# jinhan/tacotron2-vae

Measured on AMD Instinct MI355X. Metric: mel-frames/s (train step, batch=6, 80-mel), higher is better.
Workload: dtype f32; 1 GPU; configs[1]: Tacotron2-VAE fp32 train step (fwd+loss+bwd+clip+Adam), B=6/GPU fixed shape T_in=84 T_out=400, dropout on, random-init seed 1234; step_mode=hip-graph replay, decoder_forward=persistent, decoder_backward=persistent, startup_steps=43, global_batch=6, parallelism=dp1

## Files before the change

### include/t2vae.h

```cpp
#ifndef T2VAE_H
#define T2VAE_H
#include <stdint.h>
#ifdef __cplusplus
extern "C" {
#endif

#define T2V_OK 0
#define T2V_ERR_DIMS -1
#define T2V_ERR_ARG -2
#define T2V_ERR_LAUNCH -3

const char* t2v_version(void);
const char* t2v_last_error(void);

void t2v_set_phase_profile(unsigned long long* dev_buf32);
int t2v_stamp(unsigned long long* dev_buf, int slot, void* stream);
int t2v_debug_spin(int wgs, int microseconds, void* stream);

typedef struct t2v_step_params {
    uint64_t epoch;
    float lr;
    float bc1;
    float bc2s;
    float kl_weight;
// ... 208 lines not shown

typedef struct t2v_dec_items {
    int32_t* stop_item;
    const uint64_t* item_seeds;
} t2v_dec_items;
int t2v_decoder_infer_steps_items(const t2v_dec_weights* w, const t2v_dec_infer_bufs* s, int B, int T_in,
                                  int t_begin, int t_end, float gate_threshold, float p_prenet,
                                  int external_prenet, uint64_t seed, const t2v_dec_items* items, void* stream);
int t2v_decoder_infer_persistent_items(const t2v_dec_persist_weights* w, const t2v_dec_persist_bufs* s, int B, int T_in,
                                       int t_end, float gate_threshold, float p_prenet, uint64_t seed,
                                       const t2v_dec_items* items, void* stream);

typedef struct t2v_dec_window {
    int32_t back;
    int32_t ahead;
} t2v_dec_window;
int t2v_decoder_infer_steps_window(const t2v_dec_weights* w, const t2v_dec_infer_bufs* s, int B, int T_in,
                                   int t_begin, int t_end, float gate_threshold, float p_prenet,
                                   int external_prenet, uint64_t seed, const t2v_dec_items* items,
                                   const t2v_dec_window* window, void* stream);
int t2v_decoder_infer_persistent_window(const t2v_dec_persist_weights* w, const t2v_dec_persist_bufs* s, int B, int T_in,
                                        int t_end, float gate_threshold, float p_prenet, uint64_t seed,
                                        const t2v_dec_items* items, const t2v_dec_window* window, void* stream);

int t2v_conv1d_stat_blocks(int B, int T, int Cin, int Cout, int KS);
int t2v_conv1d_stat_blocks_bf16(int B, int T, int Cin, int Cout, int KS);
long long t2v_conv1d_staged_launches(void);
int t2v_conv1d_fwd(const float* W, const float* X, const float* bias, float* Y, float* stat_part,
                   int B, int Cin, int T, int Cout, int KS, void* stream);
int t2v_conv1d_dw_scratch_floats(int B, int Cin, int T, int Cout, int KS);
int t2v_conv1d_bwd(const float* W, const float* X, const float* dY, float* dX, float* dW, float* Wt_scratch,
                   float* dw_scratch,
                   int B, int Cin, int T, int Cout, int KS, void* stream);
int t2v_conv1d_flip_weights(const float* const* W, float* const* Wt, const int* Cout, const int* Cin, int KS, int n,
                            void* stream);
int t2v_conv1d_fwd_bf16(const float* W, const float* X, const float* bias, float* Y, float* stat_part,
                        void* Wp_scratch, int B, int Cin, int T, int Cout, int KS, void* stream);
int t2v_conv1d_bwd_bf16(const float* W, const float* X, const float* dY, float* dX, float* dW,
                        void* Wp_scratch, float* dw_scratch, int B, int Cin, int T, int Cout, int KS, void* stream);

int t2v_bn_act_fwd(const float* y, const float* stat_part, int nblk, const float* gamma, const float* beta,
                   float* running_mean, float* running_var, float* mean_out, float* rstd_out, float* out,
                   int B, int M, int T, int act, int training, float p_drop, float momentum, float eps,
                   uint64_t seed, uint32_t rng_stream, uint32_t rng_t, void* stream);
int t2v_bn_act_fwd_len(const float* y, const float* gamma, const float* beta, const float* running_mean,
                       const float* running_var, float* out, const int32_t* lengths, int B, int M, int T, int act, float eps,
                       void* stream);
int t2v_bn_act_bwd(const float* y, const float* dout, const float* mean, const float* rstd,
                   const float* gamma, const float* beta, float* dy, float* dgamma, float* dbeta,
                   float* dconv_bias, int B, int M, int T, int act, float p_drop, uint64_t seed,
                   uint32_t rng_stream, uint32_t rng_t, void* stream);
int t2v_bn_act_bwd_eval(const float* y, const float* dout, const float* mean, const float* rstd,
                   const float* gamma, const float* beta, float* dy, float* dgamma, float* dbeta,
                   float* dconv_bias, int B, int M, int T, int act, float p_drop, uint64_t seed,
                   uint32_t rng_stream, uint32_t rng_t, void* stream);
int t2v_bn_act_slices(int backward, int B, int M, int T, int training, int has_partials);

int t2v_embedding_fwd(const long long* ids, const float* W, float* out_bct, int B, int T, int C, int n_symbols, void* stream);
int t2v_embedding_bwd(const long long* ids, const float* dy_bct, float* dW, int B, int T, int C, int n_symbols, void* stream);

int t2v_gemm_epilogue_bwd(const float* dy, const float* y, float* out, size_t n, float scale, void* stream);

long t2v_colsum_scratch_floats(long M, long N);
int t2v_colsum(const float* A, long lda, long M, long N, float* scratch, float* out, void* stream);

int t2v_mask_outputs(float* mel, float* mel_post, float* gate, const int* lengths, int B, int C, int T, float gate_fill,
                     void* stream);
int t2v_mask_time(const float* x, float* out, const int32_t* lengths, int B, int C, int T, void* stream);
int t2v_reparam_fwd(const float* eps, const float* mu, const float* logvar, float* z, long n, void* stream);
int t2v_reparam_bwd(const float* dz, const float* eps, const float* logvar, float* dlogvar, long n, void* stream);
int t2v_gather_words(const void* const* src, void* const* dst, int n, void* stream);
int t2v_concat2_rows(const float* a, long lda, int na, const float* b, long ldb, int nb, float* out, long rows, void* stream);

int t2v_bilstm_fwd(const float* gx, const float* whh, const int32_t* lengths, float* y, float* gates,
                   float* cells, float* hx_scratch, uint32_t* sync3, int B, int T, void* stream);
int t2v_bilstm_bwd(const float* whh, const int32_t* lengths, const float* dy, const float* gates,
                   const float* cells, float* dg, float* dgx_scratch, uint32_t* sync3, int B, int T,
                   void* stream);

int t2v_gemm_f32(const float* A, long sAi, long sAk, const float* B, long sBj, long sBk, const float* bias,
                 float* C, int ldc, int M, int N, int K, int relu, int accumulate, float p_drop,
                 uint64_t seed, uint32_t rng_stream, uint32_t rng_t, void* stream);
long t2v_gemm_splitk_scratch_floats(int M, int N, int K);
int t2v_gemm_f32_splitk(const float* A, long sAi, long sAk, const float* B, long sBj, long sBk, const float* bias,
                        float* C, int ldc, int M, int N, int K, int relu, int accumulate, float p_drop,
                        uint64_t seed, uint32_t rng_stream, uint32_t rng_t, float* splitk_scratch, void* stream);

int t2v_gemm_f32_set_mode(int x3);

typedef struct t2v_gemm_group {
    const float* A;
    long sAi;
    long sAk;
    int nb;
    const float* B[3];
    long sBj[3];
    long sBk[3];
    int N[3];
    float* C[3];
    int ldc[3];
} t2v_gemm_group;
long t2v_gemm_f32_grouped_scratch_floats(const t2v_gemm_group* groups, int ngroups, int M, int K);
int t2v_gemm_f32_grouped(const t2v_gemm_group* groups, int ngroups, int M, int K, int accumulate, float* scratch, void* stream);
long t2v_gemm_f32_grouped_group_offset(const t2v_gemm_group* groups, int ngroups, int M, int K, int g);
int t2v_gemm_f32_grouped_handed(const t2v_gemm_group* groups, int ngroups, int M, int K, int accumulate, float* scratch, int handed,
                                const uint32_t* done_ctr, int done_cap, void* stream);
long t2v_gemm_bf16_grouped_scratch_floats(const t2v_gemm_group* groups, int ngroups, int M, int K);
int t2v_gemm_bf16_grouped(const t2v_gemm_group* groups, int ngroups, int M, int K, int accumulate, float* scratch, void* stream);

int t2v_conv1d_x3_set_mode(int mode);
int t2v_conv1d_takes_x3(int B, int Cin, int T, int Cout, int KS, int bf16);
#define T2V_CONV_OP_FWD 0
#define T2V_CONV_OP_DX 1
#define T2V_CONV_OP_DW 2
#define T2V_CONV_ROUTE_GEMM 0
#define T2V_CONV_ROUTE_FWD 1
#define T2V_CONV_ROUTE_FWD_DMA 2
#define T2V_CONV_ROUTE_X3 3
#define T2V_CONV_ROUTE_BF16 4
#define T2V_CONV_ROUTE_BF16K32 5
#define T2V_CONV_ROUTE_PLANE1 6
#define T2V_CONV_ROUTE_DW 7
#define T2V_CONV_ROUTE_DW_BF16 8
#define T2V_CONV_ROUTES 9
int t2v_conv1d_route(int op, int B, int Cin, int T, int Cout, int KS, int bf16, int w_mod16, int* fallback, int* tile, int* ksplit,
                     int* dw_splits, int* stat_blocks, int* dw_scratch_floats, int* plane_splits, int* plane_chunk);
const char* t2v_conv1d_route_name(int route);

int t2v_gemm_f32_batched(const float* A, long sAb, long sAi, long sAk, const float* B, long sBb, long sBj, long sBk,
                         float* C, long sCb, int ldc, int nbatch, int M, int N, int K, void* stream);
int t2v_gemm_bf16(const float* A, long sAi, long sAk, const float* B, long sBj, long sBk, const float* bias,
                  float* C, int ldc, int M, int N, int K, int relu, int accumulate, float p_drop,
                  uint64_t seed, uint32_t rng_stream, uint32_t rng_t, void* stream);
long t2v_gemm_bf16_splitk_scratch_floats(int M, int N, int K);
int t2v_gemm_bf16_splitk(const float* A, long sAi, long sAk, const float* B, long sBj, long sBk, const float* bias,
                         float* C, int ldc, int M, int N, int K, int relu, int accumulate, float p_drop,
                         uint64_t seed, uint32_t rng_stream, uint32_t rng_t, float* splitk_scratch, void* stream);

#define T2V_GEMM_ROUTE_F32_64 0
#define T2V_GEMM_ROUTE_F32_64_SPLITK 1
#define T2V_GEMM_ROUTE_F32_BIG_128 2
#define T2V_GEMM_ROUTE_F32_BIG_64 3
#define T2V_GEMM_ROUTE_F32_X3 4
#define T2V_GEMM_ROUTE_BF16_64 5
#define T2V_GEMM_ROUTE_BF16_64_SPLITK 6
#define T2V_GEMM_ROUTE_BF16_BIG 7
#define T2V_GEMM_ROUTE_BF16_BIG_SPLITK 8
#define T2V_GEMM_ROUTE_BF16_PLANES 9
#define T2V_GEMM_ROUTE_BF16_TO_F32_BIG 10
#define T2V_GEMM_ROUTES 11
int t2v_gemm_route(int M, int N, int K, long sAi, long sAk, long sBj, long sBk, int a_mod16, int b_mod16, int scratch_mod16,
                   int has_scratch, int relu, float p_drop, int bf16, int* form, int* splits, int* k_per_split);
const char* t2v_gemm_route_name(int route);


int t2v_conv2d_s2_fwd(const float* x, const float* w, const float* bias, float* y, int B, int Cx, int H, int W,
                      int Cout, int coord, void* stream);
int t2v_conv2d_s2_dw_scratch_floats(int B, int Cx, int H, int W, int Cout, int coord);
int t2v_conv2d_s2_bwd(const float* x, const float* w, const float* dy, float* dx, float* dw, float* dw_scratch,
                      int B, int Cx, int H, int W, int Cout, int coord, void* stream);

long t2v_conv2d_s2_gemm_scratch_floats(int B, int Cx, int H, int W, int Cout, int coord);
int t2v_conv2d_s2_fwd_gemm(const float* x, const float* w, const float* bias, float* y, float* scratch, int B, int Cx, int H, int W,
                           int Cout, int coord, void* stream);
int t2v_conv2d_s2_bwd_gemm(const float* x, const float* w, const float* dy, float* dx, float* dw, float* scratch, int B, int Cx, int H,
                           int W, int Cout, int coord, void* stream);
int t2v_gru_fwd(const float* gi, const float* whh, const float* bhh, float* hs, float* gsave, float* xchg,
                uint32_t* sync2, int B, int T, void* stream);
int t2v_gru_bwd(const float* whh, const float* hs, const float* gsave, const float* dh_last, float* dgi,
                float* dgh, float* xchg, uint32_t* sync2, int B, int T, void* stream);

int t2v_conv2d_s2_fwd_ragged(const float* x, const float* w, const float* bias, float* y, const int32_t* hlen, int B, int Cx,
                             int H, int W, int Cout, int coord, int x_tstride, void* stream);
long t2v_conv2d_s2_gemm_ragged_scratch_floats(int B, int Cx, int H, int W, int Cout, int coord);
int t2v_conv2d_s2_fwd_gemm_ragged(const float* x, const float* w, const float* bias, float* y, float* scratch,
                                  const int32_t* hlen, int B, int Cx, int H, int W, int Cout, int coord, int x_tstride,
                                  void* stream);
int t2v_gru_fwd_len(const float* gi, const float* whh, const float* bhh, float* hs, float* gsave, float* xchg,
                    uint32_t* sync2, const int32_t* steps, float* h_last, int B, int T, void* stream);
int t2v_loss_fwd_bwd(const float* mel, const float* post, const float* mel_t, const float* gate,
                     const float* gate_t, const float* mu, const float* logvar, float* dmel, float* dpost,
                     float* dgate, float* dmu, float* dlogvar, float* part192, float* out4, uint32_t* ticket,
                     uint64_t n_mel, int n_gate, int n_lat, float kl_weight, void* stream);

int t2v_clip_adam_step(float* params, float* grads, float* exp_avg, float* exp_avg_sq, uint64_t n,
                       float lr, float beta1, float beta2, float eps, float weight_decay,
                       float max_norm, float inv_world, float bc1, float bc2, float* partials,
                       float* norm_out, void* stream);
int t2v_clip_adam_step_guarded(float* params, float* grads, float* exp_avg, float* exp_avg_sq, uint64_t n,
                               float lr, float beta1, float beta2, float eps, float weight_decay,
                               float max_norm, float inv_world, float bc1, float bc2, float* partials,
                               float* norm_out, const uint32_t* guard, int guard_n, void* stream);
int t2v_clip_adam_ema_step_guarded(float* params, float* grads, float* exp_avg, float* exp_avg_sq, uint64_t n,
                                   float lr, float beta1, float beta2, float eps, float weight_decay,
                                   float max_norm, float inv_world, float bc1, float bc2, float* partials,
                                   float* norm_out, const uint32_t* guard, int guard_n, float* ema, float ema_rate,
                                   int ema_warmup, uint64_t ema_t, void* stream);

int t2v_mel_frontend(const float* wav_f32, const int16_t* wav_i16, const int64_t* n_samples, int B,
                     int n_stride, float scale, int n_fft, int hop, int n_mel, const float* window,
                     const float* tw512, const float* tw1024, const int32_t* mel_start,
                     const int32_t* mel_len, const float* mel_w, int maxw, float* mel_out,
                     int t_stride, void* stream);

int t2v_stft_polar(const float* wav, const int64_t* n_samples, int B, int n_stride, int n_fft, int hop,
                   const float* window, const float* tw512, const float* tw1024, float* mag, float* phase,
                   int t_stride, void* stream);
size_t t2v_istft_scratch_bytes(int B, int t_stride);
int t2v_istft(const float* mag, const float* phase, const int32_t* n_frames, int B, int t_stride, int n_fft, int hop,
              const float* window, const float* tw512, const float* tw1024, void* scratch, float* out, int out_stride,
              void* stream);
size_t t2v_griffin_lim_scratch_bytes(int B, int t_stride);
int t2v_griffin_lim(const float* mag, const float* angles, const int32_t* n_frames, int B, int t_stride, int n_fft,
                    int hop, int n_iters, const float* window, const float* tw512, const float* tw1024, void* scratch,
                    float* out, int out_stride, void* stream);
int t2v_mel_to_magnitude(const float* mel, const float* pinv_basis, const int32_t* n_frames, int B, int t_stride,
                         int n_mel, float* mag, void* stream);
size_t t2v_griffin_lim_fast_scratch_bytes(int B, int t_stride);
int t2v_griffin_lim_fast(const float* mag, const float* angles, const int32_t* n_frames, int B, int t_stride, int n_fft,
                         int hop, int n_iters, float momentum, const float* window, const float* tw512,
                         const float* tw1024, void* scratch, float* out, int out_stride, void* stream);
int t2v_mel_to_magnitude_nnls(const float* mel, const float* pinv_basis, const int32_t* tap_lo, const float* tap_w0,
                              const float* tap_w1, const int32_t* filt_start, const int32_t* filt_len, float lipschitz,
                              int n_iters, const int32_t* n_frames, int B, int t_stride, int n_mel, float* mag,
                              void* stream);

#define T2V_DTW_MAX_FRAMES 2048
size_t t2v_mel_dtw_scratch_bytes(int B, int tx_max, int ty_max);
int t2v_mel_dtw(const float* X, const int32_t* nx, int x_stride, const float* Y, const int32_t* ny, int y_stride,
                int B, int n_mel, float* dist, void* scratch, void* stream);

#define T2V_TSNE_MAX_POINTS 16384
#define T2V_TSNE_EXAG_ITERS 250
size_t t2v_tsne_scratch_bytes(int N, int D);
int t2v_tsne_affinities(const float* X, int N, int D, float perplexity, float* P, void* scratch, void* stream);
int t2v_tsne_gradient(const float* P, const float* Y, int N, float exaggeration, float* grad, float* kl_or_null,
                      void* scratch, void* stream);
int t2v_tsne_run(const float* P, float* Y_inout, int N, int n_iter, float learning_rate, float* kl_trace, void* scratch,
                 void* stream);

#define T2V_F0_MAX_LAG 400
int t2v_f0_yin(const float* y, const int32_t* n, int y_stride, int B, int tau_min, int tau_max, float threshold, float* f0,
               float* aperiodicity, int out_stride, void* stream);

#define T2V_ALIGN_FRAMES 16
size_t t2v_alignment_scratch_bytes(int B, int N, int T_in);
int t2v_alignment_stats(const float* A, long long a_stride_b, long long a_stride_t, const int32_t* n_frames,
                        const int32_t* n_text, int B, int N, int T_in, int max_jump, float cover_min, int32_t* path,
                        int path_stride, float* mass, int mass_stride, float* focus, int32_t* stats, void* scratch,
                        void* stream);

#define T2V_RESAMPLE_MAX_TAPS 32768
int t2v_resample(const void* x, int x_is_pcm16, float scale, const int32_t* n, int x_stride, int B, const float* taps, int up,
                 int down, int half, float* y, int out_stride, void* stream);
int t2v_trim_bounds(const float* y, const int32_t* n, int y_stride, int B, float top_db, int pad_frames, float* ms, int ms_stride,
                    int32_t* bounds, void* stream);
int t2v_crop_rows(const float* y, int y_stride, const int32_t* bounds, int B, void* out, int out_is_pcm16, int out_stride,
                  int32_t* stats, void* stream);

#define T2V_LATENT_MAX_POINTS 16384
#define T2V_LATENT_MAX_CLASSES 8
#define T2V_LATENT_MAX_K 32
#define T2V_LATENT_TILE 128
size_t t2v_latent_scratch_bytes(int N, int M, int C, int k, int slice_rows);
int t2v_latent_neighbours(const float* R, const int32_t* labels, int N, int D, int C, const float* Q, int M,
                          const int32_t* exclude, const int32_t* target, int k, int slice_rows, int32_t* nn_idx,
                          float* nn_dist, float* class_sum, int32_t* class_cnt, int32_t* rank, void* scratch, void* stream);

#define T2V_NCEP 13
#define T2V_ALIGNED_COUNTS 4
#define T2V_ALIGNED_SUMS 8
int t2v_mel_cepstrum(const float* M, const int32_t* n, int m_stride, int B, int n_mel, int n_cep, const float* table, float* out,
                     int out_stride, void* stream);
size_t t2v_cep_dtw_scratch_bytes(int B, int tx_max, int ty_max);
int t2v_cep_dtw_forward(const float* X, const int32_t* nx, int x_stride, const float* Y, const int32_t* ny, int y_stride, int B,
                        int n_cep, float* dist, void* scratch, void* stream);
int t2v_cep_dtw_walk(const int32_t* nx, int x_stride, const int32_t* ny, int y_stride, int B, const void* scratch, int32_t* K,
                     int32_t* path, int path_stride, void* stream);
int t2v_cep_dtw_path(const float* X, const int32_t* nx, int x_stride, const float* Y, const int32_t* ny, int y_stride, int B,
                     int n_cep, float* dist, int32_t* K, int32_t* path, int path_stride, void* scratch, void* stream);
int t2v_path_scores(const int32_t* path, const int32_t* K, int path_stride, const float* X, const int32_t* nx, int x_stride,
                    const float* Y, const int32_t* ny, int y_stride, const float* fx, int fx_stride, const float* fy, int fy_stride,
                    int B, int n_cep, int32_t* counts, float* sums, void* stream);

#define T2V_LOUDNESS_CHUNK 64
#define T2V_LOUDNESS_TILE 16384
size_t t2v_loudness_scratch_bytes(int B, int y_stride, int hop);
int t2v_loudness(const float* y, const int32_t* n, int y_stride, int B, const double* table, int hop, float* frame_ms,
                 int ms_stride, float* block_pw, int blk_stride, int32_t* rows, void* scratch, void* stream);
int t2v_scale_rows(float* y, const int32_t* n, int y_stride, int B, const float* gains, void* stream);

#define T2V_TSM_BINS 513
#define T2V_TSM_MAX_RATIO 1023
#define T2V_TSM_MAX_FRAMES (1 << 20)
size_t t2v_phase_vocoder_scratch_bytes(int B, int out_stride, int phase_lock);
int t2v_phase_vocoder(const float* mag, const float* phase, const int32_t* n_frames, int B, int T, int t_stride, int num, int den,
                      int phase_lock, float* mag_out, float* phase_out, int out_stride, void* scratch, void* stream);

size_t t2v_spsi_scratch_bytes(int B, int t_stride);
int t2v_spsi(const float* mag, const int32_t* n_frames, int B, int T, int t_stride, float* phase_out, void* scratch, void* stream);

#define T2V_ENV_BINS 513
#define T2V_ENV_MAX_ORDER 256
#define T2V_ENV_MAX_ITERS 32
int t2v_spectral_envelope(const float* mag, const int32_t* n_frames, int B, int T, int t_stride, int order, int iters, int p, int q,
                          float* log_env_out, float* mag_out, int out_stride, void* stream);
// ... 26 lines not shown
```

### tacotron2-vae_amd/csrc/gemm.hip

```cpp
#include <stdlib.h>
#include <string.h>
#include "t2v_common.h"
#include "t2v_kernels.h"
#include "t2v_coop.h"
#include "t2v_x3.h"
#include "t2v_xchg.h"
#include "gemm_x3_tile.h"

#define GM_BM 64
#define GM_BN 64
#define GM_BK 32

struct GemmArgs {
    const float* A; const float* B; const float* bias; float* C;
    long sAi, sAk, sBj, sBk;
    int M, N, K, ldc;
    int relu, accumulate;
    float p_drop; uint64_t seed; uint32_t rng_stream, rng_t;
    const t2v_step_params* step;
    int kz_chunk;
    float* part;
    int nbatch;
    long sAb, sBb, sCb;
    int nsub;
    long sAs, sBs;
    int bias_row;
    unsigned* tile_ctr;
};

__device__ __forceinline__ void gemm64_epilogue(const GemmArgs& a, f32x16& acc, int i0, int j0, int wm, int wn, int lane, int tid) {
    const int j = j0 + 32 * wn + (lane & 31);
    if (a.part) {
        if (j < a.N) {
#pragma unroll
            for (int r = 0; r < 16; ++r) {
                const int i = i0 + 32 * wm + (r & 3) + 8 * (r >> 2) + 4 * (lane >> 5);
                if (i < a.M) st_sc1(a.part + ((size_t)blockIdx.z * a.M + i) * a.N + j, acc[r]);
            }
        }
        __shared__ unsigned last_;
        asm volatile("s_waitcnt vmcnt(0)" ::: "memory");
        __syncthreads();
        unsigned* ctr = a.tile_ctr + blockIdx.y * gridDim.x + blockIdx.x;
        if (tid == 0) last_ = __hip_atomic_fetch_add(ctr, 1u, __ATOMIC_RELAXED, __HIP_MEMORY_SCOPE_AGENT) == gridDim.z - 1 ? 1u : 0u;
        __syncthreads();
        if (!last_) return;
        if (tid == 0) __hip_atomic_store(ctr, 0u, __ATOMIC_RELAXED, __HIP_MEMORY_SCOPE_AGENT);
        const int nz = (int)gridDim.z;
#pragma unroll
        for (int r = 0; r < 16; ++r) acc[r] = 0.f;
        if (j < a.N) {
            for (int z0 = 0; z0 < nz; z0 += 4) {
                float v[4][16];
#pragma unroll
                for (int u = 0; u < 4; ++u) {
                    const int z = min(z0 + u, nz - 1);
#pragma unroll
                    for (int r = 0; r < 16; ++r) {
                        const int i = min(i0 + 32 * wm + (r & 3) + 8 * (r >> 2) + 4 * (lane >> 5), a.M - 1);
                        v[u][r] = ld_sc1(a.part + ((size_t)z * a.M + i) * a.N + j);
                    }
                }
#pragma unroll
                for (int u = 0; u < 4; ++u)
                    if (z0 + u < nz) {
#pragma unroll
                        for (int r = 0; r < 16; ++r) acc[r] += v[u][r];
                    }
            }
        }
    }
    if (j < a.N) {
        const float bv = (a.bias && !a.bias_row) ? a.bias[j] : 0.f;
#pragma unroll
        for (int r = 0; r < 16; ++r) {
            const int i = i0 + 32 * wm + (r & 3) + 8 * (r >> 2) + 4 * (lane >> 5);
            if (i < a.M) {
                const size_t idx = (size_t)i * a.ldc + j;
                float v = acc[r] + ((a.bias && a.bias_row) ? a.bias[i] : bv);
                if (a.accumulate) v += a.C[idx];
                if (a.relu) v = fmaxf(v, 0.f);
                if (a.p_drop > 0.f) v *= t2v_drop_scale(t2v_step_seed(a.seed, a.step), a.rng_stream, a.rng_t, (uint32_t)idx, a.p_drop);
                a.C[idx] = v;
            }
        }
    }
}

template <bool A_KC, bool B_KC>
__global__ __launch_bounds__(256) void k_gemm_f32(GemmArgs a) {
    __shared__ float As[2][GM_BK][GM_BM + 1];
    __shared__ float Bs[2][GM_BK][GM_BN + 1];
    const int tid = threadIdx.x, wave = tid >> 6, lane = tid & 63;
    const int wm = wave >> 1, wn = wave & 1;
    const int i0 = blockIdx.y * GM_BM, j0 = blockIdx.x * GM_BN;
    if (a.nbatch > 1) {
        const int zb = a.nsub > 1 ? blockIdx.z / a.nsub : blockIdx.z, zs = a.nsub > 1 ? blockIdx.z - zb * a.nsub : 0;
        a.A += zb * a.sAb + zs * a.sAs; a.B += zb * a.sBb + zs * a.sBs; a.C += blockIdx.z * a.sCb;
    }
    const int kbeg = a.kz_chunk ? blockIdx.z * a.kz_chunk : 0, kend = a.kz_chunk ? min(a.K, kbeg + a.kz_chunk) : a.K;
    constexpr int NE = GM_BM * GM_BK / 256;
    float ra[NE], rb[NE];
    auto load_tiles = [&](int k0) {
#pragma unroll
        for (int e8 = 0; e8 < NE; ++e8) {
            const int e = tid + 256 * e8;
            {
                const int kk = A_KC ? (e & (GM_BK - 1)) : (e >> 6);
                const int ii = A_KC ? (e >> 5) : (e & (GM_BM - 1));
                const int i = i0 + ii, k = k0 + kk;
                ra[e8] = (i < a.M && k < kend) ? a.A[(long)i * a.sAi + (long)k * a.sAk] : 0.f;
            }
            {
                const int kk = B_KC ? (e & (GM_BK - 1)) : (e >> 6);
                const int jj = B_KC ? (e >> 5) : (e & (GM_BN - 1));
                const int j = j0 + jj, k = k0 + kk;
                rb[e8] = (j < a.N && k < kend) ? a.B[(long)j * a.sBj + (long)k * a.sBk] : 0.f;
            }
        }
    };
    auto store_tiles = [&](int buf) {
#pragma unroll
        for (int e8 = 0; e8 < NE; ++e8) {
            const int e = tid + 256 * e8;
            if (A_KC) As[buf][e & (GM_BK - 1)][e >> 5] = ra[e8]; else As[buf][e >> 6][e & (GM_BM - 1)] = ra[e8];
            if (B_KC) Bs[buf][e & (GM_BK - 1)][e >> 5] = rb[e8]; else Bs[buf][e >> 6][e & (GM_BN - 1)] = rb[e8];
        }
    };
    f32x16 acc;
#pragma unroll
    for (int r = 0; r < 16; ++r) acc[r] = 0.f;
    const int nkt = (kend - kbeg + GM_BK - 1) / GM_BK;
    load_tiles(kbeg);
    store_tiles(0);
    __syncthreads();
    const int ai = 32 * wm + (lane & 31), bj = 32 * wn + (lane & 31), kh = lane >> 5;
    for (int kt = 0; kt < nkt; ++kt) {
        const int buf = kt & 1;
        if (kt + 1 < nkt) load_tiles(kbeg + (kt + 1) * GM_BK);
#pragma unroll
        for (int s = 0; s < GM_BK / 2; ++s)
            acc = __builtin_amdgcn_mfma_f32_32x32x2f32(As[buf][2 * s + kh][ai], Bs[buf][2 * s + kh][bj], acc, 0, 0, 0);
        if (kt + 1 < nkt) store_tiles(buf ^ 1);
        __syncthreads();
    }
    gemm64_epilogue(a, acc, i0, j0, wm, wn, lane, tid);
}

#include "t2v_ring.h"
#define GM_CTR_RING ((size_t)1 << 16)
unsigned* t2v_arrival_counters(int tiles) {
    static T2VRing<unsigned, GM_CTR_RING, GM_CTR_RING, true> ring;
    return ring.take((size_t)tiles);
}
static int gemm_splits(int M, int N, int K) {
    const long tiles = (long)((M + GM_BM - 1) / GM_BM) * ((N + GM_BN - 1) / GM_BN);
    static const int wide = getenv("T2V_GEMM_SPLIT_POLICY") ? atoi(getenv("T2V_GEMM_SPLIT_POLICY")) : 1;
    if (wide) {
        if (tiles > 256 || K < 8 * GM_BK) return 1;
        long ns2 = (512 + tiles - 1) / tiles;
        const long maxk2 = K / (4 * GM_BK);
        if (ns2 > maxk2) ns2 = maxk2;
        if (ns2 > 32) ns2 = 32;
        return ns2 < 2 ? 1 : (int)ns2;
    }
    if (tiles >= 256 || K < 16 * GM_BK) return 1;
    long ns = 512 / tiles;
    const long maxk = K / (8 * GM_BK);
    if (ns > maxk) ns = maxk;
    if (ns > 32) ns = 32;
    return ns < 2 ? 1 : (int)ns;
}
static bool gemm_x3_shape_ok(int M, int N, int K);
static long gemm_x3_scratch_floats(int M, int N, int K, int np);
static int gemm_x3_mode();
extern "C" long t2v_gemm_splitk_scratch_floats(int M, int N, int K) {
    if (M < 1 || N < 1 || K < 1) return 0;
    if (gemm_x3_mode() && gemm_x3_shape_ok(M, N, K)) return gemm_x3_scratch_floats(M, N, K, 3);
    const int ns = gemm_splits(M, N, K);
    return ns > 1 ? (long)ns * M * N : 0;
}

#define GB_BM 128
#define GB_BK 32
#define GB_LD 160
template <bool A_KC, bool B_KC, int BN>
__global__ __launch_bounds__(256) void k_gemm_f32_big(GemmArgs a) {
    constexpr int NY = BN / 64;
    constexpr int NA = GB_BM * GB_BK / 4 / 256;
    constexpr int NB = BN * GB_BK / 4 / 256;
    constexpr int KQ = GB_BK / 4;
    __shared__ __attribute__((aligned(16))) float As[2][GB_BK][GB_LD];
    __shared__ __attribute__((aligned(16))) float Bs[2][GB_BK][BN + 32];
    const int tid = threadIdx.x, wave = tid >> 6, lane = tid & 63;
    const int wm = wave >> 1, wn = wave & 1;
    int by_ = blockIdx.y, bx_ = blockIdx.x;
    {
        const int nb = gridDim.x * gridDim.y, bid = blockIdx.y * gridDim.x + blockIdx.x;
        const int q = nb >> 3, r = nb & 7, xcd = bid & 7, idx = bid >> 3;
        const int lin = (xcd < r ? xcd * (q + 1) : r * (q + 1) + (xcd - r) * q) + idx;
        by_ = lin / gridDim.x;
        bx_ = lin - by_ * gridDim.x;
    }
    const int i0 = by_ * GB_BM, j0 = bx_ * BN;
    float4 ra[NA], rb[NB];
    auto load_tiles = [&](int k0) {
#pragma unroll
        for (int e = 0; e < NA; ++e) {
            if (A_KC) {
                const int i = min(i0 + tid / KQ + (256 / KQ) * e, a.M - 1), k = min(k0 + 4 * (tid % KQ), a.K - 4);
                ra[e] = *(const float4*)(a.A + (long)i * a.sAi + k);
            } else {
                const int k = min(k0 + (tid >> 5) + 8 * e, a.K - 1), i = min(i0 + 4 * (tid & 31), a.M - 4);
                ra[e] = *(const float4*)(a.A + (long)k * a.sAk + i);
            }
        }
#pragma unroll
        for (int e = 0; e < NB; ++e) {
            if (B_KC) {
                const int j = min(j0 + tid / KQ + (256 / KQ) * e, a.N - 1), k = min(k0 + 4 * (tid % KQ), a.K - 4);
                rb[e] = *(const float4*)(a.B + (long)j * a.sBj + k);
            } else {
                constexpr int RQ = BN / 4;
                const int k = min(k0 + tid / RQ + (256 / RQ) * e, a.K - 1), j = min(j0 + 4 * (tid % RQ), a.N - 4);
                rb[e] = *(const float4*)(a.B + (long)k * a.sBk + j);
            }
        }
    };
    auto store_tiles = [&](int buf, int k0) {
#pragma unroll
        for (int e = 0; e < NA; ++e) {
            if (A_KC) {
                const int m = tid / KQ + (256 / KQ) * e, kk = 4 * (tid % KQ);
                const float z = k0 + kk < a.K ? 1.f : 0.f;
                As[buf][kk + 0][m] = ra[e].x * z; As[buf][kk + 1][m] = ra[e].y * z;
                As[buf][kk + 2][m] = ra[e].z * z; As[buf][kk + 3][m] = ra[e].w * z;
            } else {
                const int kk = (tid >> 5) + 8 * e;
                const float z = k0 + kk < a.K ? 1.f : 0.f;
                *(float4*)&As[buf][kk][4 * (tid & 31)] = make_float4(ra[e].x * z, ra[e].y * z, ra[e].z * z, ra[e].w * z);
            }
        }
#pragma unroll
        for (int e = 0; e < NB; ++e) {
            if (B_KC) {
                const int n = tid / KQ + (256 / KQ) * e, kk = 4 * (tid % KQ);
                const float z = k0 + kk < a.K ? 1.f : 0.f;
                Bs[buf][kk + 0][n] = rb[e].x * z; Bs[buf][kk + 1][n] = rb[e].y * z;
                Bs[buf][kk + 2][n] = rb[e].z * z; Bs[buf][kk + 3][n] = rb[e].w * z;
            } else {
                constexpr int RQ = BN / 4;
                const int kk = tid / RQ + (256 / RQ) * e;
                const float z = k0 + kk < a.K ? 1.f : 0.f;
                *(float4*)&Bs[buf][kk][4 * (tid % RQ)] = make_float4(rb[e].x * z, rb[e].y * z, rb[e].z * z, rb[e].w * z);
            }
        }
    };
    f32x16 acc[2][NY];
#pragma unroll
    for (int x = 0; x < 2; ++x)
#pragma unroll
        for (int y = 0; y < NY; ++y)
#pragma unroll
            for (int r = 0; r < 16; ++r) acc[x][y][r] = 0.f;
    const int nkt = (a.K + GB_BK - 1) / GB_BK;
    load_tiles(0);
    store_tiles(0, 0);
    __syncthreads();
    const int am = 64 * wm + (lane & 31), bn = (BN / 2) * wn + (lane & 31), kh = lane >> 5;
    for (int kt = 0; kt < nkt; ++kt) {
        const int buf = kt & 1;
        if (kt + 1 < nkt) load_tiles((kt + 1) * GB_BK);
#pragma unroll
        for (int h = 0; h < 2; ++h) {
            float av[GB_BK / 4][2], bw[GB_BK / 4][NY];
#pragma unroll
            for (int s = 0; s < GB_BK / 4; ++s) {
                const int kr = GB_BK / 2 * h + 2 * s + kh;
                av[s][0] = As[buf][kr][am];
                av[s][1] = As[buf][kr][am + 32];
#pragma unroll
                for (int y = 0; y < NY; ++y) bw[s][y] = Bs[buf][kr][bn + 32 * y];
            }
            __builtin_amdgcn_sched_barrier(0);
#pragma unroll
            for (int s = 0; s < GB_BK / 4; ++s) {
#pragma unroll
                for (int y = 0; y < NY; ++y) {
                    acc[0][y] = __builtin_amdgcn_mfma_f32_32x32x2f32(av[s][0], bw[s][y], acc[0][y], 0, 0, 0);
                    acc[1][y] = __builtin_amdgcn_mfma_f32_32x32x2f32(av[s][1], bw[s][y], acc[1][y], 0, 0, 0);
                }
            }
        }
        if (kt + 1 < nkt) store_tiles(buf ^ 1, (kt + 1) * GB_BK);
        __syncthreads();
    }
    const uint64_t seed = t2v_step_seed(a.seed, a.step);
// ... 547 lines not shown
            if (gr[g].N[p] < GX_BN || (gr[g].N[p] % GX_BN)) return false;
            tiles += (long)(gr[g].N[p] / GX_BN) * ((M + GX_BM - 1) / GX_BM);
        }
    return tiles >= 64;
}
static int gemm_grouped_impl(const t2v_gemm_group* gr, int ngroups, int M, int K, int accumulate, float* scratch, void* stream_, int np,
                             int handed = -1, const uint32_t* done_ctr = nullptr, int done_cap = 0) {
    hipStream_t stream = (hipStream_t)stream_;
    if (!gr || ngroups < 1 || ngroups > 2 || M < 1 || K < 1) return T2V_ERR_ARG;
    for (int g = 0; g < ngroups; ++g) {
        if (!gr[g].A || gr[g].nb < 1 || gr[g].nb > 3) return T2V_ERR_ARG;
        for (int p = 0; p < gr[g].nb; ++p)
            if (!gr[g].B[p] || !gr[g].C[p] || gr[g].N[p] < 1 || gr[g].ldc[p] < gr[g].N[p]) return T2V_ERR_ARG;
    }
    if (handed >= 0 && (handed >= ngroups || !done_ctr || done_cap < 0 || np != 3 || !scratch || ((uintptr_t)scratch & 15) ||
                        !gemm_grouped_x3_ok(gr, ngroups, M, K, np)))
        return T2V_ERR_ARG;
    if (!scratch || ((uintptr_t)scratch & 15) || !gemm_grouped_x3_ok(gr, ngroups, M, K, np)) {
        for (int g = 0; g < ngroups; ++g)
            for (int p = 0; p < gr[g].nb; ++p) {
                const int rc = (np == 3 ? t2v_gemm_f32 : t2v_gemm_bf16)(gr[g].A, gr[g].sAi, gr[g].sAk, gr[g].B[p], gr[g].sBj[p], gr[g].sBk[p], nullptr, gr[g].C[p], gr[g].ldc[p],
                                            M, gr[g].N[p], K, 0, accumulate, 0.f, 0, 0, 0, stream_);
                if (rc != T2V_OK) return rc;
            }
        return T2V_OK;
    }
    const long G = gx_groups(K, np), RpA = gx_rp(M);
    GemmX3Args a;
    a.nprod = ngroups;
    uint4* at = (uint4*)scratch;
    int tile0 = 0;
    for (int g = 0; g < ngroups; ++g) {
        GemmX3Prod& P = a.pr[g];
        long n = 0;
        for (int p = 0; p < gr[g].nb; ++p) n += gr[g].N[p];
        P.Ap = at; at += gx_plane_slots(M, K, np);
        P.Bp = at; at += np * G * n;
        P.RpA = RpA; P.RpB = n; P.N = (int)n; P.tiles_x = (int)(n / GX_BN); P.tile0 = tile0; P.nseg = gr[g].nb;
        if (g != handed) gx_split_launch(gr[g].A, gr[g].sAi, gr[g].sAk, M, K, (uint4*)P.Ap, RpA, G, 0, stream, np);
        long col = 0;
        for (int p = 0; p < 3; ++p) {
            const int q = p < gr[g].nb ? p : gr[g].nb - 1;
            P.seg_col[p] = p < gr[g].nb ? (int)col : 0x7fffffff; P.segC[p] = gr[g].C[q]; P.seg_ldc[p] = gr[g].ldc[q];
            if (p < gr[g].nb) {
                if (g != handed) gx_split_launch(gr[g].B[p], gr[g].sBj[p], gr[g].sBk[p], gr[g].N[p], K, (uint4*)P.Bp, n, G, col, stream, np);
                col += gr[g].N[p];
            }
        }
        tile0 += P.tiles_x * (int)((M + GX_BM - 1) / GX_BM);
    }
    if (ngroups == 1) a.pr[1] = a.pr[0];
    a.ntiles = tile0;
    a.G = G; a.bias = nullptr; a.M = M; a.relu = 0; a.accumulate = accumulate;
    a.p_drop = 0.f; a.seed = 0; a.rng_stream = 0; a.rng_t = 0; a.step = t2v_step_for(stream);
    a.st_chunk = 0; a.part = nullptr; a.tile_ctr = nullptr;
    a.done_ctr = handed >= 0 ? done_ctr : nullptr; a.done_prod = handed >= 0 ? handed : 0; a.done_cap = (unsigned)done_cap;
    if (np == 3) k_gemm_x3p<3, 2><<<dim3(a.ntiles, 1, 1), 256, 0, stream>>>(a);
    else k_gemm_x3p<1, GX_NG1><<<dim3(a.ntiles, 1, 1), 256, 0, stream>>>(a);
    return t2v_check_launch();
}
extern "C" int t2v_gemm_f32_grouped(const t2v_gemm_group* gr, int ngroups, int M, int K, int accumulate, float* scratch, void* stream_) {
    return gemm_grouped_impl(gr, ngroups, M, K, accumulate, scratch, stream_, 3);
}
extern "C" int t2v_gemm_f32_grouped_handed(const t2v_gemm_group* gr, int ngroups, int M, int K, int accumulate, float* scratch, int handed,
                                           const uint32_t* done_ctr, int done_cap, void* stream_) {
    if (handed < 0) return T2V_ERR_ARG;
    return gemm_grouped_impl(gr, ngroups, M, K, accumulate, scratch, stream_, 3, handed, done_ctr, done_cap);
}
extern "C" long t2v_gemm_f32_grouped_group_offset(const t2v_gemm_group* gr, int ngroups, int M, int K, int g) {
    if (!gr || ngroups < 1 || ngroups > 2 || g < 0 || g >= ngroups || M < 1 || K < 1 || !gemm_grouped_x3_ok(gr, ngroups, M, K, 3)) return -1;
    return g == 0 ? 0 : gemm_grouped_scratch(gr, 1, M, K, 3);
}
extern "C" int t2v_gemm_bf16_grouped(const t2v_gemm_group* gr, int ngroups, int M, int K, int accumulate, float* scratch, void* stream_) {
    return gemm_grouped_impl(gr, ngroups, M, K, accumulate, scratch, stream_, 1);
}

__global__ __launch_bounds__(256) void k_epilogue_bwd(const float4* __restrict__ dy, const float4* __restrict__ y,
                                                      float4* __restrict__ out, size_t n4, float scale) {
    const size_t i = (size_t)blockIdx.x * 256 + threadIdx.x;
    if (i >= n4) return;
    const float4 g = dy[i], v = y[i];
    float4 o;
    o.x = v.x != 0.f ? g.x * scale : 0.f; o.y = v.y != 0.f ? g.y * scale : 0.f;
    o.z = v.z != 0.f ? g.z * scale : 0.f; o.w = v.w != 0.f ? g.w * scale : 0.f;
    out[i] = o;
}
__global__ __launch_bounds__(256) void k_epilogue_bwd_tail(const float* __restrict__ dy, const float* __restrict__ y,
                                                           float* __restrict__ out, size_t lo, size_t n, float scale) {
    const size_t i = lo + threadIdx.x;
    if (i < n) out[i] = y[i] != 0.f ? dy[i] * scale : 0.f;
}

extern "C" int t2v_gemm_epilogue_bwd(const float* dy, const float* y, float* out, size_t n, float scale, void* stream_) {
    hipStream_t stream = (hipStream_t)stream_;
    if (!dy || !y || !out || n < 1) return T2V_ERR_ARG;
    if (((uintptr_t)dy | (uintptr_t)y | (uintptr_t)out) & 15) return T2V_ERR_ARG;
    const size_t n4 = n / 4;
    if (n4) k_epilogue_bwd<<<(unsigned)((n4 + 255) / 256), 256, 0, stream>>>((const float4*)dy, (const float4*)y, (float4*)out, n4, scale);
    if (n & 3) k_epilogue_bwd_tail<<<1, 256, 0, stream>>>(dy, y, out, 4 * n4, n, scale);
    return t2v_check_launch();
}

extern "C" int t2v_gemm_f32(const float* A, long sAi, long sAk, const float* B, long sBj, long sBk, const float* bias,
                            float* C, int ldc, int M, int N, int K, int relu, int accumulate, float p_drop,
                            uint64_t seed, uint32_t rng_stream, uint32_t rng_t, void* stream_);
static int gemm_bf16_impl(const float* A, long sAi, long sAk, const float* B, long sBj, long sBk, const float* bias,
                          float* C, int ldc, int M, int N, int K, int relu, int accumulate, float p_drop,
                          uint64_t seed, uint32_t rng_stream, uint32_t rng_t, float* splitk_scratch, void* stream_);
extern "C" int t2v_gemm_bf16(const float* A, long sAi, long sAk, const float* B, long sBj, long sBk, const float* bias,
                             float* C, int ldc, int M, int N, int K, int relu, int accumulate, float p_drop,
                             uint64_t seed, uint32_t rng_stream, uint32_t rng_t, void* stream_) {
    return gemm_bf16_impl(A, sAi, sAk, B, sBj, sBk, bias, C, ldc, M, N, K, relu, accumulate, p_drop, seed, rng_stream, rng_t, nullptr, stream_);
}
extern "C" int t2v_gemm_bf16_splitk(const float* A, long sAi, long sAk, const float* B, long sBj, long sBk, const float* bias,
                                    float* C, int ldc, int M, int N, int K, int relu, int accumulate, float p_drop,
                                    uint64_t seed, uint32_t rng_stream, uint32_t rng_t, float* splitk_scratch, void* stream_) {
    return gemm_bf16_impl(A, sAi, sAk, B, sBj, sBk, bias, C, ldc, M, N, K, relu, accumulate, p_drop, seed, rng_stream, rng_t, splitk_scratch, stream_);
}
static int gemm_bf16_impl(const float* A, long sAi, long sAk, const float* B, long sBj, long sBk, const float* bias,
                          float* C, int ldc, int M, int N, int K, int relu, int accumulate, float p_drop,
                          uint64_t seed, uint32_t rng_stream, uint32_t rng_t, float* splitk_scratch, void* stream_) {
    hipStream_t stream = (hipStream_t)stream_;
    if (!A || !B || !C || M < 1 || N < 1 || K < 1 || ldc < N) return T2V_ERR_ARG;
    GemmArgs a;
    a.A = A; a.B = B; a.bias = bias; a.C = C; a.sAi = sAi; a.sAk = sAk; a.sBj = sBj; a.sBk = sBk;
    a.M = M; a.N = N; a.K = K; a.ldc = ldc; a.relu = relu; a.accumulate = accumulate;
    a.p_drop = p_drop; a.seed = seed; a.rng_stream = rng_stream; a.rng_t = rng_t; a.step = t2v_step_for(stream);
    a.kz_chunk = 0; a.part = nullptr; a.nbatch = 1; a.sAb = a.sBb = a.sCb = 0; a.nsub = 1; a.sAs = a.sBs = 0; a.bias_row = 0; a.tile_ctr = nullptr;
    const GemmRoute rt = gemm_route_bf16(gemm_shape_of(a, splitk_scratch));
    if (rt.route == T2V_GEMM_ROUTE_BF16_PLANES) return gemm_x3_run(a, splitk_scratch, stream, rt, 1);
    if (rt.route == T2V_GEMM_ROUTE_BF16_TO_F32_BIG)
        return t2v_gemm_f32(A, sAi, sAk, B, sBj, sBk, bias, C, ldc, M, N, K, relu, accumulate, p_drop, seed, rng_stream, rng_t, stream_);
    const bool big = rt.route == T2V_GEMM_ROUTE_BF16_BIG || rt.route == T2V_GEMM_ROUTE_BF16_BIG_SPLITK;
    const int bm = big ? GBB_BM : GM_BM, bn = big ? GBB_BN : GM_BN;
    dim3 grid((N + bn - 1) / bn, (M + bm - 1) / bm, rt.splits);
    if (rt.splits > 1) {
        a.kz_chunk = rt.chunk;
        a.part = splitk_scratch;
        a.tile_ctr = t2v_arrival_counters((int)(grid.x * grid.y));
        if (!a.tile_ctr) return T2V_ERR_LAUNCH;
    }
    const bool akc = rt.form & 1, bkc = (rt.form & 2) != 0;
    if (big) {
        if (akc && bkc) k_gemm_bf16_big_rr<true, true><<<grid, 256, 0, stream>>>(a);
        else if (akc) k_gemm_bf16_big_rr<true, false><<<grid, 256, 0, stream>>>(a);
        else if (bkc) k_gemm_bf16_big_rr<false, true><<<grid, 256, 0, stream>>>(a);
        else k_gemm_bf16_big_rr<false, false><<<grid, 256, 0, stream>>>(a);
        return t2v_check_launch();
    }
    if (akc && bkc) k_gemm_bf16<true, true><<<grid, 256, 0, stream>>>(a);
    else if (akc) k_gemm_bf16<true, false><<<grid, 256, 0, stream>>>(a);
    else if (bkc) k_gemm_bf16<false, true><<<grid, 256, 0, stream>>>(a);
    else k_gemm_bf16<false, false><<<grid, 256, 0, stream>>>(a);
    return t2v_check_launch();
}

static int gemm_f32_impl(const float* A, long sAi, long sAk, const float* B, long sBj, long sBk, const float* bias,
                         float* C, int ldc, int M, int N, int K, int relu, int accumulate, float p_drop,
                         uint64_t seed, uint32_t rng_stream, uint32_t rng_t, float* splitk_scratch, void* stream_);
extern "C" int t2v_gemm_f32(const float* A, long sAi, long sAk, const float* B, long sBj, long sBk, const float* bias,
                            float* C, int ldc, int M, int N, int K, int relu, int accumulate, float p_drop,
                            uint64_t seed, uint32_t rng_stream, uint32_t rng_t, void* stream_) {
    return gemm_f32_impl(A, sAi, sAk, B, sBj, sBk, bias, C, ldc, M, N, K, relu, accumulate, p_drop, seed, rng_stream, rng_t,
                         nullptr, stream_);
}
extern "C" int t2v_gemm_f32_splitk(const float* A, long sAi, long sAk, const float* B, long sBj, long sBk, const float* bias,
                                   float* C, int ldc, int M, int N, int K, int relu, int accumulate, float p_drop,
                                   uint64_t seed, uint32_t rng_stream, uint32_t rng_t, float* splitk_scratch, void* stream_) {
    return gemm_f32_impl(A, sAi, sAk, B, sBj, sBk, bias, C, ldc, M, N, K, relu, accumulate, p_drop, seed, rng_stream, rng_t,
                         splitk_scratch, stream_);
}
static int gemm_f32_impl(const float* A, long sAi, long sAk, const float* B, long sBj, long sBk, const float* bias,
                         float* C, int ldc, int M, int N, int K, int relu, int accumulate, float p_drop,
                         uint64_t seed, uint32_t rng_stream, uint32_t rng_t, float* splitk_scratch, void* stream_) {
    hipStream_t stream = (hipStream_t)stream_;
    if (!A || !B || !C || M < 1 || N < 1 || K < 1 || ldc < N) return T2V_ERR_ARG;
    GemmArgs a;
    a.A = A; a.B = B; a.bias = bias; a.C = C; a.sAi = sAi; a.sAk = sAk; a.sBj = sBj; a.sBk = sBk;
    a.M = M; a.N = N; a.K = K; a.ldc = ldc; a.relu = relu; a.accumulate = accumulate;
    a.p_drop = p_drop; a.seed = seed; a.rng_stream = rng_stream; a.rng_t = rng_t; a.step = t2v_step_for(stream);
    a.kz_chunk = 0; a.part = nullptr; a.nbatch = 1; a.sAb = a.sBb = a.sCb = 0; a.nsub = 1; a.sAs = a.sBs = 0; a.bias_row = 0; a.tile_ctr = nullptr;
    const GemmRoute rt = gemm_route_f32(gemm_shape_of(a, splitk_scratch));
    const bool akc = rt.form & 1, bkc = (rt.form & 2) != 0;
    if (rt.route == T2V_GEMM_ROUTE_F32_X3) return gemm_x3_run(a, splitk_scratch, stream, rt);
    if (rt.route == T2V_GEMM_ROUTE_F32_BIG_128 || rt.route == T2V_GEMM_ROUTE_F32_BIG_64) {
        const bool wide = rt.route == T2V_GEMM_ROUTE_F32_BIG_128;
        const int BN = wide ? 128 : 64;
        dim3 gb((N + BN - 1) / BN, (M + GB_BM - 1) / GB_BM);
#define T2V_BIG(AK, BK)                                                             \
        if (wide) k_gemm_f32_big<AK, BK, 128><<<gb, 256, 0, stream>>>(a);           \
        else k_gemm_f32_big<AK, BK, 64><<<gb, 256, 0, stream>>>(a)
        if (akc && bkc) { T2V_BIG(true, true); }
        else if (akc) { T2V_BIG(true, false); }
        else if (bkc) { T2V_BIG(false, true); }
        else { T2V_BIG(false, false); }
#undef T2V_BIG
        return t2v_check_launch();
    }
    dim3 grid((N + GM_BN - 1) / GM_BN, (M + GM_BM - 1) / GM_BM, rt.splits);
    if (rt.splits > 1) {
        a.kz_chunk = rt.chunk;
        a.part = splitk_scratch;
        a.tile_ctr = t2v_arrival_counters((int)(grid.x * grid.y));
        if (!a.tile_ctr) return T2V_ERR_LAUNCH;
    }
    if (akc && bkc) k_gemm_f32<true, true><<<grid, 256, 0, stream>>>(a);
    else if (akc) k_gemm_f32<true, false><<<grid, 256, 0, stream>>>(a);
    else if (bkc) k_gemm_f32<false, true><<<grid, 256, 0, stream>>>(a);
    else k_gemm_f32<false, false><<<grid, 256, 0, stream>>>(a);
    return t2v_check_launch();
}

int t2v_gemm_f32_batched_ex(const float* A, long sAb, long sAs, long sAi, long sAk, const float* B, long sBb, long sBs, long sBj, long sBk,
                            const float* bias_row, float* C, long sCb, int ldc, int nbatch, int nsub, int M, int N, int K, hipStream_t stream) {
    if (!A || !B || !C || nbatch < 1 || nsub < 1 || (long)nbatch * nsub > 65535 || M < 1 || N < 1 || K < 1 || ldc < N) return T2V_ERR_ARG;
    GemmArgs a;
    a.A = A; a.B = B; a.bias = bias_row; a.C = C; a.sAi = sAi; a.sAk = sAk; a.sBj = sBj; a.sBk = sBk;
    a.M = M; a.N = N; a.K = K; a.ldc = ldc; a.relu = 0; a.accumulate = 0;
    a.p_drop = 0.f; a.seed = 0; a.rng_stream = 0; a.rng_t = 0; a.step = t2v_step_for(stream);
    a.kz_chunk = 0; a.part = nullptr; a.nbatch = nbatch * nsub > 1 ? nbatch * nsub : 1; a.sAb = sAb; a.sBb = sBb; a.sCb = sCb;
    a.nsub = nsub; a.sAs = sAs; a.sBs = sBs; a.bias_row = bias_row ? 1 : 0; a.tile_ctr = nullptr;
    const bool akc = sAk == 1, bkc = sBk == 1;
    dim3 grid((N + GM_BN - 1) / GM_BN, (M + GM_BM - 1) / GM_BM, nbatch * nsub);
    if (akc && bkc) k_gemm_f32<true, true><<<grid, 256, 0, stream>>>(a);
    else if (akc) k_gemm_f32<true, false><<<grid, 256, 0, stream>>>(a);
    else if (bkc) k_gemm_f32<false, true><<<grid, 256, 0, stream>>>(a);
    else k_gemm_f32<false, false><<<grid, 256, 0, stream>>>(a);
    return t2v_check_launch();
}
extern "C" int t2v_gemm_f32_batched(const float* A, long sAb, long sAi, long sAk, const float* B, long sBb, long sBj, long sBk,
                                    float* C, long sCb, int ldc, int nbatch, int M, int N, int K, void* stream_) {
    return t2v_gemm_f32_batched_ex(A, sAb, 0, sAi, sAk, B, sBb, 0, sBj, sBk, nullptr, C, sCb, ldc, nbatch, 1, M, N, K, (hipStream_t)stream_);
}
```

Measured before the change: 230,600 mel-frames/s.

## Add register-staged, vectorized double-buffered f32 64x64 GEMM kernel

Adds a new f32 64x64 MFMA GEMM kernel that keeps two register staging slots, so global loads for tile k+2 are issued while tile k is computed and tile k+1 is stored to LDS. It uses float4 vectorized loads when alignment and strides allow, padded LDS leading dimensions, and a lighter lgkmcnt barrier. All non-big f32 GEMM launches (plain, split-K and batched) are routed through it by default, falling back to the old kernel only when offsets would overflow. It uses more registers, which may lower occupancy, and adds an optional JSON logging path and a launch counter.

Result: no change. 231,300 mel-frames/s, median of 6 (+0.3%).

```diff
diff --git a/include/t2vae.h b/include/t2vae.h
--- a/include/t2vae.h
+++ b/include/t2vae.h
@@ -384,6 +384,7 @@
 int t2v_gemm_route(int M, int N, int K, long sAi, long sAk, long sBj, long sBk, int a_mod16, int b_mod16, int scratch_mod16,
                    int has_scratch, int relu, float p_drop, int bf16, int* form, int* splits, int* k_per_split);
 const char* t2v_gemm_route_name(int route);
+long long t2v_gemm64_staged_launches(void);
 
 
 int t2v_conv2d_s2_fwd(const float* x, const float* w, const float* bias, float* y, int B, int Cx, int H, int W,
diff --git a/tacotron2-vae_amd/csrc/gemm.hip b/tacotron2-vae_amd/csrc/gemm.hip
--- a/tacotron2-vae_amd/csrc/gemm.hip
+++ b/tacotron2-vae_amd/csrc/gemm.hip
@@ -1,5 +1,8 @@
+#include <stdio.h>
 #include <stdlib.h>
 #include <string.h>
+#include <atomic>
+#include <type_traits>
 #include "t2v_common.h"
 #include "t2v_kernels.h"
 #include "t2v_coop.h"
@@ -143,6 +146,124 @@
             acc = __builtin_amdgcn_mfma_f32_32x32x2f32(As[buf][2 * s + kh][ai], Bs[buf][2 * s + kh][bj], acc, 0, 0, 0);
         if (kt + 1 < nkt) store_tiles(buf ^ 1);
         __syncthreads();
+    }
+    gemm64_epilogue(a, acc, i0, j0, wm, wn, lane, tid);
+}
+
+#define GM_RING 2
+template <bool KC, bool VEC>
+struct Gm64Stage {
+    static constexpr int LD = KC ? GM_BM + 1 : GM_BM + 4;
+    const float* p;
+    int sr, sk;
+    int rows;
+    int kend, K;
+    __device__ __forceinline__ void load(float (&R)[8], int k0, int tid) const {
+        if constexpr (VEC && KC) {
+            const int kc = min(k0 + 4 * (tid & 7), K - 4);
+#pragma unroll
+            for (int q = 0; q < 2; ++q) {
+                const float4 v = *(const float4*)(p + min((tid >> 3) + 32 * q, rows - 1) * sr + kc);
+                R[4 * q] = v.x; R[4 * q + 1] = v.y; R[4 * q + 2] = v.z; R[4 * q + 3] = v.w;
+            }
+        } else if constexpr (VEC) {
+            const int ic = min(4 * (tid & 15), rows - 4);
+#pragma unroll
+            for (int q = 0; q < 2; ++q) {
+                const float4 v = *(const float4*)(p + min(k0 + (tid >> 4) + 16 * q, kend - 1) * sk + ic);
+                R[4 * q] = v.x; R[4 * q + 1] = v.y; R[4 * q + 2] = v.z; R[4 * q + 3] = v.w;
+            }
+        } else {
+#pragma unroll
+            for (int e8 = 0; e8 < 8; ++e8) {
+                const int e = tid + 256 * e8;
+                const int kk = KC ? (e & (GM_BK - 1)) : (e >> 6), ii = KC ? (e >> 5) : (e & (GM_BM - 1));
+                R[e8] = p[min(ii, rows - 1) * sr + min(k0 + kk, kend - 1) * sk];
+            }
+        }
+    }
+    __device__ __forceinline__ void store(float* S, const float (&R)[8], int k0, int tid) const {
+        const bool inner = rows >= GM_BM && k0 + GM_BK <= kend;
+        if constexpr (VEC && KC) {
+#pragma unroll
+            for (int q = 0; q < 2; ++q) {
+                const int r = (tid >> 3) + 32 * q, kk = 4 * (tid & 7);
+                const bool ok = inner || (r < rows && k0 + kk < kend);
+#pragma unroll
+                for (int o = 0; o < 4; ++o) S[(kk + o) * LD + r] = ok ? R[4 * q + o] : 0.f;
+            }
+        } else if constexpr (VEC) {
+#pragma unroll
+            for (int q = 0; q < 2; ++q) {
+                const int kk = (tid >> 4) + 16 * q, i4 = 4 * (tid & 15);
+                const bool ok = inner || (i4 < rows && k0 + kk < kend);
+                *(float4*)&S[kk * LD + i4] = ok ? make_float4(R[4 * q], R[4 * q + 1], R[4 * q + 2], R[4 * q + 3]) : make_float4(0.f, 0.f, 0.f, 0.f);
+            }
+        } else {
+#pragma unroll
+            for (int e8 = 0; e8 < 8; ++e8) {
+                const int e = tid + 256 * e8;
+                const int kk = KC ? (e & (GM_BK - 1)) : (e >> 6), ii = KC ? (e >> 5) : (e & (GM_BM - 1));
+                S[kk * LD + ii] = (inner || (ii < rows && k0 + kk < kend)) ? R[e8] : 0.f;
+            }
+        }
+    }
+};
+__device__ __forceinline__ void gm64_lds_barrier() { asm volatile("s_waitcnt lgkmcnt(0)\n\ts_barrier" ::: "memory"); }
+
+template <bool A_KC, bool B_KC, bool A_VEC, bool B_VEC>
+__global__ __launch_bounds__(256) void k_gemm_f32_st(GemmArgs a) {
+    using SA = Gm64Stage<A_KC, A_VEC>;
+    using SB = Gm64Stage<B_KC, B_VEC>;
+    __shared__ __attribute__((aligned(16))) float As[2][GM_BK * SA::LD];
+    __shared__ __attribute__((aligned(16))) float Bs[2][GM_BK * SB::LD];
+    const int tid = threadIdx.x, wave = tid >> 6, lane = tid & 63;
+    const int wm = wave >> 1, wn = wave & 1;
+    const int i0 = blockIdx.y * GM_BM, j0 = blockIdx.x * GM_BN;
+    if (a.nbatch > 1) {
+        const int zb = a.nsub > 1 ? blockIdx.z / a.nsub : blockIdx.z, zs = a.nsub > 1 ? blockIdx.z - zb * a.nsub : 0;
+        a.A += zb * a.sAb + zs * a.sAs; a.B += zb * a.sBb + zs * a.sBs; a.C += blockIdx.z * a.sCb;
+    }
+    const int kbeg = a.kz_chunk ? blockIdx.z * a.kz_chunk : 0, kend = a.kz_chunk ? min(a.K, kbeg + a.kz_chunk) : a.K;
+    const int nkt = (kend - kbeg + GM_BK - 1) / GM_BK;
+    f32x16 acc;
+#pragma unroll
+    for (int r = 0; r < 16; ++r) acc[r] = 0.f;
+    if (nkt > 0) {
+        const SA sa{a.A + (long)i0 * a.sAi, (int)a.sAi, (int)a.sAk, a.M - i0, kend, a.K};
+        const SB sb{a.B + (long)j0 * a.sBj, (int)a.sBj, (int)a.sBk, a.N - j0, kend, a.K};
+        float ra[GM_RING][8], rb[GM_RING][8];
+        const int ai = 32 * wm + (lane & 31), bj = 32 * wn + (lane & 31), kh = lane >> 5;
+        auto load_tiles = [&](int slot, int t) {
+            const int k0 = kbeg + min(t, nkt - 1) * GM_BK;
+            sa.load(ra[slot], k0, tid); sb.load(rb[slot], k0, tid);
+            __builtin_amdgcn_sched_barrier(0);
+        };
+        auto store_tiles = [&](int buf, int slot, int t) {
+            const int k0 = kbeg + min(t, nkt - 1) * GM_BK;
+            sa.store(As[buf], ra[slot], k0, tid); sb.store(Bs[buf], rb[slot], k0, tid);
+        };
+        auto mfma_tile = [&](const float* SAp, const float* SBp) {
+#pragma unroll
+            for (int s = 0; s < GM_BK / 2; ++s)
+                acc = __builtin_amdgcn_mfma_f32_32x32x2f32(SAp[(2 * s + kh) * SA::LD + ai], SBp[(2 * s + kh) * SB::LD + bj], acc, 0, 0, 0);
+        };
+        load_tiles(0, 0);
+        load_tiles(1, 1);
+        store_tiles(0, 0, 0);
+        gm64_lds_barrier();
+        int kt = 0;
+        for (; kt + 1 < nkt; kt += 2) {
+            load_tiles(0, kt + 2);
+            mfma_tile(As[0], Bs[0]);
+            store_tiles(1, 1, kt + 1);
+            gm64_lds_barrier();
+            load_tiles(1, kt + 3);
+            mfma_tile(As[1], Bs[1]);
+            store_tiles(0, 0, kt + 2);
+            gm64_lds_barrier();
+        }
+        if (kt < nkt) mfma_tile(As[0], Bs[0]);
     }
     gemm64_epilogue(a, acc, i0, j0, wm, wn, lane, tid);
 }
@@ -996,6 +1117,53 @@
     else if (akc) k_gemm_bf16<true, false><<<grid, 256, 0, stream>>>(a);
     else if (bkc) k_gemm_bf16<false, true><<<grid, 256, 0, stream>>>(a);
     else k_gemm_bf16<false, false><<<grid, 256, 0, stream>>>(a);
+    return t2v_check_launch();
+}
+
+static std::atomic<long long> g_gemm64_staged_launches{0};
+extern "C" long long t2v_gemm64_staged_launches(void) { return g_gemm64_staged_launches.load(std::memory_order_relaxed); }
+static bool gemm64_operand_vec(bool kc, const float* p, long s_row, long s_k, int rows, int K, long s_batch, long s_sub) {
+    if (((uintptr_t)p & 15) || (s_batch & 3) || (s_sub & 3)) return false;
+    return kc ? (s_k == 1 && !(s_row & 3) && !(K & 3)) : (s_row == 1 && !(s_k & 3) && !(rows & 3));
+}
+static bool gemm64_offsets_fit(long s_row, long s_k, int K) {
+    return s_row >= 0 && s_k >= 0 && (double)GM_BM * (double)s_row + (double)K * (double)s_k < 2147483648.0;
+}
+static void gemm64_log(const GemmArgs& a, bool akc, bool bkc, dim3 grid, bool staged, bool av, bool bv) {
+    static FILE* const f = getenv("T2V_GEMM64_LOG") ? fopen(getenv("T2V_GEMM64_LOG"), "a") : nullptr;
+    if (!f) return;
+    fprintf(f, "{\"M\":%d,\"N\":%d,\"K\":%d,\"sAi\":%ld,\"sAk\":%ld,\"sBj\":%ld,\"sBk\":%ld,\"form\":\"%c%c\",\"splits\":%d,\"kz_chunk\":%d,"
+            "\"nbatch\":%d,\"nsub\":%d,\"sAb\":%ld,\"sBb\":%ld,\"sCb\":%ld,\"sAs\":%ld,\"sBs\":%ld,\"ldc\":%d,\"a_mod16\":%d,\"b_mod16\":%d,"
+            "\"bias\":%d,\"bias_row\":%d,\"relu\":%d,\"accumulate\":%d,\"p_drop\":%g,\"grid\":[%u,%u,%u],\"staged\":%d,\"a_vec\":%d,\"b_vec\":%d}\n",
+            a.M, a.N, a.K, a.sAi, a.sAk, a.sBj, a.sBk, akc ? 'k' : 'r', bkc ? 'k' : 'r', a.part ? (int)grid.z : 1, a.kz_chunk,
+            a.nbatch > 1 ? a.nbatch / a.nsub : 1, a.nsub, a.sAb, a.sBb, a.sCb, a.sAs, a.sBs, a.ldc, (int)((uintptr_t)a.A & 15), (int)((uintptr_t)a.B & 15),
+            a.bias ? 1 : 0, a.bias_row, a.relu, a.accumulate, (double)a.p_drop, grid.x, grid.y, grid.z, (int)staged, (int)av, (int)bv);
+    fflush(f);
+}
+static int gemm64_launch(const GemmArgs& a, bool akc, bool bkc, dim3 grid, hipStream_t stream) {
+    static const int staging = getenv("T2V_GEMM_STAGING") ? atoi(getenv("T2V_GEMM_STAGING")) : 1;
+    const bool staged = staging && gemm64_offsets_fit(a.sAi, a.sAk, a.K) && gemm64_offsets_fit(a.sBj, a.sBk, a.K);
+    const bool av = staged && gemm64_operand_vec(akc, a.A, a.sAi, a.sAk, a.M, a.K, a.nbatch > 1 ? a.sAb : 0, a.nbatch > 1 ? a.sAs : 0);
+    const bool bv = staged && gemm64_operand_vec(bkc, a.B, a.sBj, a.sBk, a.N, a.K, a.nbatch > 1 ? a.sBb : 0, a.nbatch > 1 ? a.sBs : 0);
+    gemm64_log(a, akc, bkc, grid, staged, av, bv);
+    if (staged) {
+#define T2V_ST(AK, BK)                                                                      \
+        if (av && bv) k_gemm_f32_st<AK, BK, true, true><<<grid, 256, 0, stream>>>(a);       \
+        else if (av) k_gemm_f32_st<AK, BK, true, false><<<grid, 256, 0, stream>>>(a);       \
+        else if (bv) k_gemm_f32_st<AK, BK, false, true><<<grid, 256, 0, stream>>>(a);       \
+        else k_gemm_f32_st<AK, BK, false, false><<<grid, 256, 0, stream>>>(a)
+        if (akc && bkc) { T2V_ST(true, true); }
+        else if (akc) { T2V_ST(true, false); }
+        else if (bkc) { T2V_ST(false, true); }
+        else { T2V_ST(false, false); }
+#undef T2V_ST
+        g_gemm64_staged_launches.fetch_add(1, std::memory_order_relaxed);
+        return t2v_check_launch();
+    }
+    if (akc && bkc) k_gemm_f32<true, true><<<grid, 256, 0, stream>>>(a);
+    else if (akc) k_gemm_f32<true, false><<<grid, 256, 0, stream>>>(a);
+    else if (bkc) k_gemm_f32<false, true><<<grid, 256, 0, stream>>>(a);
+    else k_gemm_f32<false, false><<<grid, 256, 0, stream>>>(a);
     return t2v_check_launch();
 }
 
@@ -1048,11 +1216,7 @@
         a.tile_ctr = t2v_arrival_counters((int)(grid.x * grid.y));
         if (!a.tile_ctr) return T2V_ERR_LAUNCH;
     }
-    if (akc && bkc) k_gemm_f32<true, true><<<grid, 256, 0, stream>>>(a);
-    else if (akc) k_gemm_f32<true, false><<<grid, 256, 0, stream>>>(a);
-    else if (bkc) k_gemm_f32<false, true><<<grid, 256, 0, stream>>>(a);
-    else k_gemm_f32<false, false><<<grid, 256, 0, stream>>>(a);
-    return t2v_check_launch();
+    return gemm64_launch(a, akc, bkc, grid, stream);
 }
 
 int t2v_gemm_f32_batched_ex(const float* A, long sAb, long sAs, long sAi, long sAk, const float* B, long sBb, long sBs, long sBj, long sBk,
@@ -1066,11 +1230,7 @@
     a.nsub = nsub; a.sAs = sAs; a.sBs = sBs; a.bias_row = bias_row ? 1 : 0; a.tile_ctr = nullptr;
     const bool akc = sAk == 1, bkc = sBk == 1;
     dim3 grid((N + GM_BN - 1) / GM_BN, (M + GM_BM - 1) / GM_BM, nbatch * nsub);
-    if (akc && bkc) k_gemm_f32<true, true><<<grid, 256, 0, stream>>>(a);
-    else if (akc) k_gemm_f32<true, false><<<grid, 256, 0, stream>>>(a);
-    else if (bkc) k_gemm_f32<false, true><<<grid, 256, 0, stream>>>(a);
-    else k_gemm_f32<false, false><<<grid, 256, 0, stream>>>(a);
-    return t2v_check_launch();
+    return gemm64_launch(a, akc, bkc, grid, stream);
 }
 extern "C" int t2v_gemm_f32_batched(const float* A, long sAb, long sAi, long sAk, const float* B, long sBb, long sBj, long sBk,
                                     float* C, long sCb, int ldc, int nbatch, int M, int N, int K, void* stream_) {
```
